# HSoumi/hybrid-als-twotower-recommender

Hardware: AMD Instinct MI355X
Metric: ALS epochs/sec + scored user-item pairs/sec at rank=64, 1/2/4/8 MI355X (higher is better)
Workload: dtype f64

## Files before the change

### hybrid-als-twotower-recommender_amd/csrc/als.hip

```cpp
#include "als_row.h"

namespace hrec {

template <int NT, int CH, int MODE, bool S64 = false, bool IMP = false>
__device__ __forceinline__ void als_row(int64_t row, int lane, const int64_t* __restrict__ indptr,
                                        const int32_t* __restrict__ indices, const float* __restrict__ values,
                                        const float* __restrict__ src, int64_t n_src, int k, double reg,
                                        float* __restrict__ dst, double* __restrict__ lds, double alpha = 0.0,
                                        const double* __restrict__ yty = nullptr) {
  constexpr int KP = 16 * NT;
  const int64_t beg = indptr[row];
  const int64_t end = indptr[row + 1];
  float* __restrict__ out = dst + row * KP;
  if (end == beg) {
    if (lane < KP) out[lane] = 0.f;
    return;
  }
  d4 acc[NT * (NT + 1) / 2];
  double* scratch = lds + RowLds<KP>::kUpPad;
  double* bsh = scratch + 128 + 2 * KP;
  if constexpr (IMP) {
    int n_pos = 0;
    gram_row<NT, CH, MODE, NoHook, S64, true>(beg, end, lane, indices, values, src, n_src, k, reg, acc, bsh, lds,
                                              NoHook(), alpha, yty, &n_pos);
    if (n_pos == 0) {
      if (lane < KP) out[lane] = 0.f;
      return;
    }
  } else {
    gram_row<NT, CH, MODE, NoHook, S64>(beg, end, lane, indices, values, src, n_src, k, reg, acc, bsh, lds);
  }
  factor_row<NT>(lane, acc, lds, scratch, bsh, out);
}

template <int NT, int CH, int MODE, bool S64 = false>
__global__ __launch_bounds__(64, HREC_ALS_WAVES) void als_half_sweep_f64_kernel(
    const int64_t* __restrict__ indptr, const int32_t* __restrict__ indices,
    const float* __restrict__ values, int64_t n_rows, const float* __restrict__ src, int64_t n_src,
    int k, double reg, float* __restrict__ dst) {
  __shared__ __attribute__((aligned(16))) double lds[RowLds<16 * NT>::kSize];
  als_row<NT, CH, MODE, S64>(blockIdx.x, threadIdx.x, indptr, indices, values, src, n_src, k, reg, dst, lds);
}

template <int NT, int CH>
__global__ __launch_bounds__(64, HREC_ALS_WAVES) void als_half_sweep_implicit_kernel(
    const int64_t* __restrict__ indptr, const int32_t* __restrict__ indices,
    const float* __restrict__ values, int64_t n_rows, const float* __restrict__ src, int64_t n_src,
    int k, double reg, double alpha, const double* __restrict__ yty, float* __restrict__ dst) {
  __shared__ __attribute__((aligned(16))) double lds[RowLds<16 * NT>::kSize];
  als_row<NT, CH, 0, false, true>(blockIdx.x, threadIdx.x, indptr, indices, values, src, n_src, k, reg, dst, lds,
                                  alpha, yty);
}

__global__ __launch_bounds__(256) void f32_to_f64_kernel(const float* __restrict__ in, int64_t n,
                                                         double* __restrict__ out) {
  for (int64_t i = (int64_t)blockIdx.x * 256 + threadIdx.x; i < n; i += (int64_t)gridDim.x * 256)
    out[i] = (double)in[i];
}

__global__ __launch_bounds__(256) void transpose_kernel(const float* __restrict__ in, int64_t rows,
                                                        int64_t cols, float* __restrict__ out, int64_t ld_out) {
  __shared__ float tile[64][65];
  const int64_t r0 = (int64_t)blockIdx.x * 64;
  const int64_t c0 = (int64_t)blockIdx.y * 64;
  const int tx = threadIdx.x & 63, ty = threadIdx.x >> 6;
  for (int i = ty; i < 64; i += 4) {
    const int64_t r = r0 + i, c = c0 + tx;
    tile[i][tx] = (r < rows && c < cols) ? in[r * cols + c] : 0.f;
  }
  __syncthreads();
  for (int i = ty; i < 64; i += 4) {
    const int64_t c = c0 + i, r = r0 + tx;
    if (r < rows && c < cols) out[c * ld_out + r] = tile[tx][i];
  }
}

}

using namespace hrec;

extern "C" int hrec_als_half_sweep(const int64_t* indptr, const int32_t* indices, const float* values,
                                   int64_t n_rows, const float* src_factors, int64_t n_src, int k,
                                   int kp, double reg_param, int accum_mode, float* dst_factors,
                                   void* stream) {
  HREC_REQUIRE(hrec_factor_ld_ok(kp), "als_half_sweep: kp must be 16, 32, 64, 96, 128, 192 or 256 (got %d)", kp);
  HREC_REQUIRE(k >= 1 && k <= kp, "als_half_sweep: need 1 <= k <= kp (k=%d kp=%d)", k, kp);
  HREC_REQUIRE(n_rows >= 0 && n_src >= 0, "als_half_sweep: negative size");
  HREC_REQUIRE(n_rows < 0x7fffffffll, "als_half_sweep: too many rows for one launch");
  HREC_REQUIRE(accum_mode == 0 || accum_mode == 1, "als_half_sweep: accum_mode %d unsupported", accum_mode);
  HREC_REQUIRE(reg_param >= 0.0, "als_half_sweep: reg_param must be >= 0");
  if (n_rows == 0) return HREC_OK;
  HREC_REQUIRE(indptr && dst_factors, "als_half_sweep: null pointer");
  HREC_REQUIRE(n_src > 0 && src_factors && indices && values,
               "als_half_sweep: null source factors / CSR arrays");
  HREC_REQUIRE(n_src < 0x7fffffffll, "als_half_sweep: too many source rows for one launch");
  HREC_REQUIRE(kp != 64 || n_src * (int64_t)kp * 4 <= (int64_t)0xffffffffll,
               "als_half_sweep: %lld source rows of %d floats exceed the 4 GiB a gather resource spans; shard the "
               "source side", (long long)n_src, kp);
  if (kp > 64) {
    HREC_REQUIRE(accum_mode == 0, "als_half_sweep: kp > 64 supports accum_mode 0 (f64) only");
    return hrec_als_half_sweep_wide(indptr, indices, values, n_rows, src_factors, n_src, k, kp, reg_param,
                                    dst_factors, stream);
  }
  hipStream_t s = as_stream(stream);
  const dim3 grid((unsigned)n_rows), block(64);
#define HREC_SWEEP(NT, CH, M)                                                                      \
  hipLaunchKernelGGL((als_half_sweep_f64_kernel<NT, CH, M>), grid, block, 0, s, indptr, indices, values, \
                     n_rows, src_factors, n_src, k, reg_param, dst_factors)
  if (accum_mode == 0) {
    if (kp == 64) HREC_SWEEP(4, HREC_ALS_CH0, 0);
    else if (kp == 32) HREC_SWEEP(2, 8, 0);
    else HREC_SWEEP(1, 8, 0);
  } else {
    if (kp == 64) HREC_SWEEP(4, HREC_ALS_CH1, 1);
    else if (kp == 32) HREC_SWEEP(2, 4, 1);
    else HREC_SWEEP(1, 4, 1);
  }
#undef HREC_SWEEP
  return check_launch("als_half_sweep_f64_kernel");
}

extern "C" int hrec_als_half_sweep_implicit(const int64_t* indptr, const int32_t* indices, const float* values,
                                            int64_t n_rows, const float* src_factors, int64_t n_src, int k, int kp,
                                            double reg_param, double alpha, const double* yty, float* dst_factors,
                                            void* stream) {
  HREC_REQUIRE(kp == 16 || kp == 32 || kp == 64,
               "als_half_sweep_implicit: kp must be 16, 32 or 64 (implicit feedback supports rank <= 64; got kp %d)",
// ... 12 lines not shown
               "als_half_sweep_implicit: null source factors / CSR arrays");
  hipStream_t s = as_stream(stream);
  const dim3 grid((unsigned)n_rows), block(64);
#define HREC_SWEEP(NT, CH)                                                                                  \
  hipLaunchKernelGGL((als_half_sweep_implicit_kernel<NT, CH>), grid, block, 0, s, indptr, indices, values, \
                     n_rows, src_factors, n_src, k, reg_param, alpha, yty, dst_factors)
  if (kp == 64) HREC_SWEEP(4, HREC_ALS_CH0);
  else if (kp == 32) HREC_SWEEP(2, 8);
  else HREC_SWEEP(1, 8);
#undef HREC_SWEEP
  return check_launch("als_half_sweep_implicit_kernel");
}

extern "C" int hrec_f32_to_f64(const float* in, int64_t n, double* out, void* stream) {
  HREC_REQUIRE(n >= 0, "f32_to_f64: negative size");
  if (n == 0) return HREC_OK;
  HREC_REQUIRE(in && out, "f32_to_f64: null pointer");
  int64_t blocks = (n + 255) / 256;
  if (blocks > 4096) blocks = 4096;
  hipLaunchKernelGGL(f32_to_f64_kernel, dim3((unsigned)blocks), dim3(256), 0, as_stream(stream), in, n, out);
  return check_launch("f32_to_f64_kernel");
}

extern "C" int hrec_als_half_sweep_src64(const int64_t* indptr, const int32_t* indices, const float* values,
                                         int64_t n_rows, const double* src64, int64_t n_src, int k, int kp,
                                         double reg_param, float* dst_factors, void* stream) {
  HREC_REQUIRE(kp == 64, "als_half_sweep_src64: kp must be 64 (got %d)", kp);
  HREC_REQUIRE(k >= 1 && k <= kp, "als_half_sweep_src64: need 1 <= k <= kp (k=%d kp=%d)", k, kp);
  HREC_REQUIRE(n_rows >= 0 && n_src >= 0, "als_half_sweep_src64: negative size");
  HREC_REQUIRE(n_rows < 0x7fffffffll && n_src < 0x7fffffffll, "als_half_sweep_src64: too many rows for one launch");
  HREC_REQUIRE(n_src * (int64_t)kp * 8 <= (int64_t)0xffffffffll,
               "als_half_sweep_src64: %lld f64 source rows exceed the 4 GiB a gather resource spans", (long long)n_src);
  HREC_REQUIRE(reg_param >= 0.0, "als_half_sweep_src64: reg_param must be >= 0");
  if (n_rows == 0) return HREC_OK;
  HREC_REQUIRE(indptr && dst_factors, "als_half_sweep_src64: null pointer");
  HREC_REQUIRE(n_src > 0 && src64 && indices && values, "als_half_sweep_src64: null source factors / CSR arrays");
  HREC_REQUIRE(((uintptr_t)src64 & 15) == 0, "als_half_sweep_src64: src64 must be 16-B aligned");
  hipLaunchKernelGGL((als_half_sweep_f64_kernel<4, HREC_ALS_CH0, 0, true>), dim3((unsigned)n_rows), dim3(64), 0,
                     as_stream(stream), indptr, indices, values, n_rows, reinterpret_cast<const float*>(src64), n_src,
                     k, reg_param, dst_factors);
  return check_launch("als_half_sweep_f64_kernel (f64 sources)");
}

extern "C" int hrec_transpose_f32(const float* in, int64_t rows, int64_t cols, float* out, int64_t ld_out,
                                  void* stream) {
  HREC_REQUIRE(rows >= 0 && cols >= 0, "transpose: negative size");
  HREC_REQUIRE(ld_out >= rows, "transpose: ld_out < rows");
  if (rows == 0 || cols == 0) return HREC_OK;
  HREC_REQUIRE(in && out, "transpose: null pointer");
  const dim3 grid((unsigned)((rows + 63) / 64), (unsigned)((cols + 63) / 64)), block(256);
  hipLaunchKernelGGL(transpose_kernel, grid, block, 0, as_stream(stream), in, rows, cols, out, ld_out);
  return check_launch("transpose_kernel");
}

#ifdef HREC_ALS_STAMPS
extern "C" int hrec_debug_als_stamps(unsigned long long* host_out, int reset) {
  if (hipMemcpyFromSymbol(host_out, HIP_SYMBOL(g_als_stamps), sizeof(g_als_stamps)) != hipSuccess) return -2;
  if (reset) {
    unsigned long long z[8] = {0};
    if (hipMemcpyToSymbol(HIP_SYMBOL(g_als_stamps), z, sizeof(z)) != hipSuccess) return -2;
  }
  return 0;
}
#endif
// ... 1 lines not shown
```

### hybrid-als-twotower-recommender_amd/csrc/als_row.h

```cpp
#pragma once
#include <type_traits>

#include "common.h"

#ifndef HREC_ALS_WAVES
#define HREC_ALS_WAVES 2
#endif
#ifndef HREC_ALS_CH0
#define HREC_ALS_CH0 8
#endif
#ifndef HREC_ALS_ABLATE
#define HREC_ALS_ABLATE 0
#endif
#ifndef HREC_ALS_SOLVE_UNROLL
#define HREC_ALS_SOLVE_UNROLL 8
#endif
#ifndef HREC_ALS_CH1
#define HREC_ALS_CH1 4
#endif
#ifndef HREC_ALS_INTCVT
#define HREC_ALS_INTCVT 0
#endif
#ifndef HREC_ALS_RLPANEL
#define HREC_ALS_RLPANEL 0
// ... 1 lines not shown
#ifndef HREC_ALS_DIAG4
#define HREC_ALS_DIAG4 3
#endif
#ifndef HREC_ALS_PIPE
#define HREC_ALS_PIPE 1
#endif
#ifndef HREC_ALS_PF
#define HREC_ALS_PF 8
#endif
#ifndef HREC_ALS_PF64
#define HREC_ALS_PF64 4
#endif
#ifndef HREC_ALS_PAIR8
#define HREC_ALS_PAIR8 2
#endif
#ifndef HREC_ALS_ROT1DPP
#define HREC_ALS_ROT1DPP 1
#endif
#ifndef HREC_ALS_ROT1DPP64
#define HREC_ALS_ROT1DPP64 0
#endif
#ifndef HREC_ALS_PR
#define HREC_ALS_PR 2
#endif

namespace hrec {

typedef double d4 __attribute__((ext_vector_type(4)));
typedef hrec_f4 f4;

template <int NT>
struct Vec;
template <>
struct Vec<4> {
  float x[4];
  __device__ static Vec load(const float* p) {
    const float4 t = *reinterpret_cast<const float4*>(p);
    return Vec{{t.x, t.y, t.z, t.w}};
  }
};
template <>
struct Vec<2> {
  float x[2];
  __device__ static Vec load(const float* p) {
    const float2 t = *reinterpret_cast<const float2*>(p);
    return Vec{{t.x, t.y}};
// ... 102 lines not shown
  const long long x = __double_as_longlong(v);
  const int lo = __builtin_amdgcn_readlane((int)x, src);
  const int hi = __builtin_amdgcn_readlane((int)(x >> 32), src);
  return __longlong_as_double(((long long)hi << 32) | (long long)(unsigned)lo);
}

__device__ __forceinline__ void wave_lds_sync() {
  __builtin_amdgcn_fence(__ATOMIC_RELEASE, "wavefront");
  __builtin_amdgcn_wave_barrier();
  __builtin_amdgcn_fence(__ATOMIC_ACQUIRE, "wavefront");
}

template <int KP>
struct RowLds {
  static constexpr int kUp = KP * (KP + 1) / 2;
  static constexpr int kUpPad = ((kUp > 256 ? kUp : 256) + 1) & ~1;
  static constexpr int kSize = kUpPad + 128 + 3 * KP;
};

struct NoHook {
  __device__ void operator()() const {}
};

template <int NT, int CH, int MODE, typename Hook = NoHook, bool S64 = false, bool IMP = false>
__device__ __forceinline__ void gram_row(int64_t beg, int64_t end, int lane, const int32_t* __restrict__ indices,
                                         const float* __restrict__ values, const float* __restrict__ src,
                                         int64_t n_src, int k, double reg, d4 (&acc)[NT * (NT + 1) / 2],
                                         double* __restrict__ bsh, double* __restrict__ stage,
                                         Hook before_lds = Hook(), double alpha = 0.0,
                                         const double* __restrict__ yty = nullptr, int* npos = nullptr) {
  static_assert(!IMP || (MODE == 0 && !S64), "implicit feedback: f64 accumulation of f32 sources only");
  constexpr int KP = 16 * NT;
  constexpr int NPAIR = NT * (NT + 1) / 2;
  constexpr int CHN = 4 * CH;
  const int sub = lane >> 4;
  const int col = lane & 15;
  const int64_t n = end - beg;
  int n_pos = 0;

  STAMP_DECL;
  STAMP(0);
#pragma unroll
  for (int p = 0; p < NPAIR; ++p) acc[p] = d4{0.0, 0.0, 0.0, 0.0};
  if constexpr (HREC_ALS_ABLATE == 4) {
#pragma unroll
    for (int I = 0, p = 0; I < NT; p += NT - I, ++I)
#pragma unroll
      for (int rr = 0; rr < 4; ++rr) acc[p][rr] = (sub + 4 * rr == col) ? 1.0 + reg * (double)n : 0.0;
    if (lane < KP) bsh[lane] = 1.0;
    wave_lds_sync();
    return;
  }
  f4 fa[NPAIR];
  double bp[NT];
#pragma unroll
  for (int t = 0; t < NT; ++t) bp[t] = 0.0;

  auto load_iv = [&](int64_t base, int& ii, float& vv) {
    const int64_t p = base + (lane % CHN);
    const bool ok = (lane < CHN) && (p < end);
    ii = ok ? indices[p] : -1;
    vv = ok ? values[p] : 0.f;
  };
  auto gather = [&](Vec<NT> (&buf)[CH], int ii) {
#pragma unroll
    for (int s = 0; s < CH; ++s) {
      const int idx = __shfl(ii, 4 * s + sub, kWave);
      const int safe = idx < 0 ? 0 : idx;
      Vec<NT> v = Vec<NT>::load(src + (int64_t)safe * KP + NT * col);
#pragma unroll
      for (int t = 0; t < NT; ++t) v.x[t] = idx < 0 ? 0.f : v.x[t];
      buf[s] = v;
    }
  };

  if constexpr (HREC_ALS_PIPE && NT == 4 && !IMP) {
  constexpr int PF = S64 ? HREC_ALS_PF64 : HREC_ALS_PF;
  static_assert(16 % PF == 0, "prefetch distance must divide the window");
  static_assert(!S64 || (NT == 4 && MODE == 0 && (HREC_ALS_DIAG4 == 0 || HREC_ALS_DIAG4 == 3)),
                "f64 sources: kp 64, f64 accumulation only");
  const int voff = (S64 ? 8 : 4) * NT * col;
  const int bp_addr = 4 * sub;
  const uint64_t sbase = (uint64_t)src;
  i4v rsrc;
  rsrc.x = __builtin_amdgcn_readfirstlane((int)(uint32_t)sbase);
  rsrc.y = __builtin_amdgcn_readfirstlane((int)(uint32_t)(sbase >> 32) | ((KP * (S64 ? 8 : 4)) << 16));
  rsrc.z = __builtin_amdgcn_readfirstlane((int)n_src);
  rsrc.w = 0x00020000;
  auto load_win = [&](int64_t w, int& ii, float& vv) {
    const int64_t p = beg + 64 * w + lane;
    const int64_t pc = p < end ? p : end - 1;
    const int iraw = indices[pc];
    const float vraw = values[pc];
    ii = p < end ? iraw : -1;
    vv = p < end ? vraw : 0.f;
  };
  auto bperm = [&](int win, int s) -> int { return __builtin_amdgcn_ds_bpermute(bp_addr + 16 * s, win); };
  const int64_t nsteps = (n + 3) >> 2;
  int iw0, iw1;
  float rw0, rw1;
  load_win(0, iw0, rw0);
  load_win(1, iw1, rw1);
  using RingT = std::conditional_t<S64, VecD, Vec<NT>>;
  auto ring_load = [&](int vi) -> RingT {
    if constexpr (S64) return struct_load_d(rsrc, vi, voff);
    else return struct_load<NT>(rsrc, vi, voff);
  };
  RingT ring[PF];
#pragma unroll
  for (int s = 0; s < PF; ++s) ring[s] = ring_load(bperm(iw0, s));
  int nidx = bperm(iw0, PF);
  constexpr bool kDiag4 = HREC_ALS_DIAG4 && MODE == 0;
  constexpr bool kAhead = HREC_ALS_DIAG4 == 2 && MODE == 0;
  constexpr bool kMemRot = HREC_ALS_DIAG4 == 3 && MODE == 0;
  constexpr int PR = kMemRot ? HREC_ALS_PR : 1;
  constexpr bool kRot1Dpp = kMemRot && (S64 ? HREC_ALS_ROT1DPP64 : HREC_ALS_ROT1DPP);
  static_assert(PR < PF, "rotated loads are issued from the current windows");
  const int voff1 = (S64 ? 8 : 4) * NT * ((col + 4) & 15), voff2 = (S64 ? 8 : 4) * NT * ((col + 8) & 15);
  auto rot_load = [&](int vi, int vo) -> RingT {
    if constexpr (S64) return struct_load_d(rsrc, vi, vo);
    else return struct_load<NT>(rsrc, vi, vo);
  };
  constexpr bool kPairL = kMemRot && HREC_ALS_PAIR8 == 2 && NT == 4;
  using PairT = std::conditional_t<S64, VecD2, Vec<2>>;
  const int hoff = (lane & 8) ? (S64 ? 16 : 8) : 0;
  auto pair_load = [&](int vi, int vo) -> PairT {
    if constexpr (S64) return struct_load_d2(rsrc, vi, vo);
    else return struct_load<2>(rsrc, vi, vo);
  };
  RingT rot1[PR], rot2[PR];
  PairT rotA[PR], rotB[PR];
  if constexpr (kMemRot) {
#pragma unroll
    for (int q = 0; q < PR; ++q) {
      const int vi = bperm(iw0, q);
      if constexpr (!kRot1Dpp) rot1[q] = rot_load(vi, voff1);
      if constexpr (kPairL) {
        rotA[q] = pair_load(vi, voff + hoff);
        rotB[q] = pair_load(vi, voff2 + hoff);
// ... 134 lines not shown
            }
          } else {
            fa[p] = __builtin_amdgcn_mfma_f32_16x16x4f32(cur.x[I], cur.x[J], fa[p], 0, 0, 0);
          }
          ++p;
        }
      }
#pragma unroll
      for (int t = 0; t < NT; ++t) bp[t] = fma(rv, a[t], bp[t]);
      if (MODE == 1 && ((s % HREC_ALS_CH1) == HREC_ALS_CH1 - 1 || s + 1 == rem)) {
#pragma unroll
        for (int p2 = 0; p2 < NPAIR; ++p2) {
#pragma unroll
          for (int rr = 0; rr < 4; ++rr) acc[p2][rr] += (double)fa[p2][rr];
        }
      }
    }
    if (stop || 16 * (w + 1) >= nsteps) break;
    iw0 = iw1;
    rw0 = rw1;
    iw1 = iw2;
    rw1 = rw2;
  }
  if constexpr (kDiag4) {
    const int i4 = lane >> 4, q4 = (lane >> 2) & 3, j4 = lane & 3;
#pragma unroll
    for (int I = 0, p = 0; I < NT; p += NT - I, ++I) {
#pragma unroll
      for (int sh = 0; sh < 3; ++sh) {
        const int r = 4 * q4 + i4, c = 4 * ((q4 + sh) & 3) + j4;
        if (kPair8 && sh == 2) {
          const bool mine = kPairL ? (q4 >= 2) == (I >= 2) : (q4 >= 2) == (I % 2 == 1);
          const double v = kPairL ? dc[I & 1] : dc[I / 2];
          stage[mine ? r * 16 + c : 256] = v;
          stage[mine ? c * 16 + r : 257] = v;
          continue;
        }
        stage[r * 16 + c] = dg[I][sh];
        stage[c * 16 + r] = dg[I][sh];
      }
      wave_lds_sync();
#pragma unroll
      for (int rr = 0; rr < 4; ++rr) acc[p][rr] = stage[(sub + 4 * rr) * 16 + col];
      wave_lds_sync();
    }
  }
// ... 97 lines not shown
#pragma unroll
      for (int J = I; J < NT; ++J) {
#pragma unroll
        for (int rr = 0; rr < 4; ++rr) acc[p][rr] += yty[(NT * (sub + 4 * rr) + I) * KP + NT * col + J];
        ++p;
      }
    }
    *npos = n_pos;
  }
  const double lambda = (double)(IMP ? (int64_t)n_pos : n) * reg;
  {
    int p = 0;
#pragma unroll
    for (int I = 0; I < NT; ++I) {
#pragma unroll
      for (int rr = 0; rr < 4; ++rr) {
        if (sub + 4 * rr == col) acc[p][rr] += (NT * col + I < k) ? lambda : 1.0;
      }
      p += NT - I;
    }
  }
}

template <int NT>
__device__ __forceinline__ void factor_row(int lane, d4 (&acc)[NT * (NT + 1) / 2], double* __restrict__ Up,
                                           double* __restrict__ scratch, const double* __restrict__ bsh,
                                           float* __restrict__ out) {
  constexpr int KP = 16 * NT;
  constexpr int NPAIR = NT * (NT + 1) / 2;
  double* __restrict__ colbuf = scratch;
  double* __restrict__ dsh = colbuf + 128;
  double* __restrict__ rdsh = dsh + KP;
  const int sub = lane >> 4, col = lane & 15;
  STAMP_DECL;
  STAMP(0);
  if constexpr (HREC_ALS_ABLATE == 1) {
    double sum = 0.0;
#pragma unroll
    for (int p = 0; p < NPAIR; ++p) sum += acc[p][0] + acc[p][1] + acc[p][2] + acc[p][3];
    wave_lds_sync();
    if (lane < KP) out[lane] = (float)(sum + bsh[lane]);
    return;
  }
  auto pidx = [](int I, int K) { return I * NT - (I * (I - 1)) / 2 + (K - I); };
  double bs = 0.0;
#pragma unroll
  for (int J = 0; J < NT; ++J) {
#pragma unroll
    for (int K = J; K < NT; ++K) {
#pragma unroll
      for (int rr = 0; rr < 4; ++rr) {
        const int q = 16 * J + sub + 4 * rr, c = 16 * K + col;
        if (q <= c) Up[tri(c) + q] = acc[pidx(J, K)][rr];
      }
    }
    wave_lds_sync();
    if (J == 0) bs = lane < KP ? bsh[lane] : 0.0;
    const int c = lane;
    const bool own = c >= 16 * J && c < KP;
    double a[16];
#pragma unroll
    for (int m = 0; m < 16; ++m) {
      const int q = 16 * J + m;
      if constexpr (HREC_ALS_RLPANEL) {
        a[m] = !own ? 0.0 : q <= c ? Up[tri(c) + q] : c < 16 * J + 16 ? Up[tri(q) + c] : 0.0;
      } else {
        a[m] = (own && q <= c) ? Up[tri(c) + q] : 0.0;
      }
    }
    double piv = bcast(a[0], 16 * J);
    if constexpr (HREC_ALS_RLPANEL) {
#pragma unroll
      for (int i = 0; i < 16; ++i) {
        const int pv = 16 * J + i;
        double u[16];
#pragma unroll
        for (int m0 = i + 1; m0 < 16; ++m0) u[m0] = bcast(a[m0], pv);
        const double r0 = __builtin_amdgcn_rcp(piv);
        const double r = fma(r0, fma(-piv, r0, 1.0), r0);
// ... 46 lines not shown
          if (!kRl2 || m0 > i) a[m0 + 1] = fma(-u.y, ut, a[m0 + 1]);
        }
      }
    }
    wave_lds_sync();
    if (J + 1 < NT) {
      double dq[4];
#pragma unroll
      for (int rr = 0; rr < 4; ++rr) dq[rr] = dsh[16 * J + sub + 4 * rr];
      d4 yv[NT];
#pragma unroll
      for (int K = J + 1; K < NT; ++K) {
#pragma unroll
        for (int rr = 0; rr < 4; ++rr) {
          const double x = Up[tri(16 * K + col) + 16 * J + sub + 4 * rr];
          acc[pidx(J, K)][rr] = x;
          yv[K][rr] = x * dq[rr];
        }
      }
#pragma unroll
      for (int K = J + 1; K < NT; ++K) {
#pragma unroll
        for (int M = K; M < NT; ++M) {
#pragma unroll
          for (int rr = 0; rr < 4; ++rr)
            acc[pidx(K, M)] = __builtin_amdgcn_mfma_f64_16x16x4f64(-acc[pidx(J, K)][rr], yv[M][rr],
                                                                    acc[pidx(K, M)], 0, 0, 0);
        }
      }
    }
  }
  STAMP(3);
  const int lc = lane < KP ? lane : KP - 1;
  const double myrd = rdsh[lc];
  if constexpr (HREC_ALS_ABLATE == 3) {
    if (lane < KP) out[lane] = (float)(myrd + Up[tri(lane)]);
    return;
  }
  double bi = bs * myrd;
#pragma unroll HREC_ALS_SOLVE_UNROLL
  for (int q = KP - 1; q >= 0; --q) {
    const double u = Up[tri(q) + (lane < KP ? lane : 0)];
    const double xq = bcast(bi, q);
    if (lane < q) bi = fma(-u, xq, bi);
  }
  STAMP(4);
  if (lane < KP) out[NT * (lane & 15) + (lane >> 4)] = (float)bi;
  wave_lds_sync();
}

}
```

### hybrid-als-twotower-recommender_amd/src/_hrec.py

```python
import ctypes
import os

import torch

_HERE = os.path.dirname(os.path.abspath(__file__))
LIB_PATH = os.environ.get("HREC_LIB") or os.path.join(os.path.dirname(_HERE), "lib", "libhrec.so")

_c_i32 = ctypes.c_int
_c_i64 = ctypes.c_int64
_c_u64 = ctypes.c_uint64
_c_dbl = ctypes.c_double
_c_sz = ctypes.c_size_t
_vp = ctypes.c_void_p

_SIGNATURES = {
    "hrec_abi_version": (_c_i32, []),
    "hrec_last_error": (ctypes.c_char_p, []),
    "hrec_synth_row_counts": (_c_i32, [_c_u64, _c_u64, _c_i64, _c_i64, _c_i64, _c_i32, _vp, _vp]),
    "hrec_synth_fill": (_c_i32, [_c_u64, _c_u64, _c_u64, _c_i64, _c_i64, _c_i64, _c_i32, _c_i32,
                                 _vp, _vp, _vp, _vp]),
    "hrec_scan_workspace_bytes": (_c_sz, [_c_i64]),
    "hrec_exclusive_scan_i64": (_c_i32, [_vp, _c_i64, _vp, _vp, _c_sz, _vp]),
    "hrec_encode_ids_workspace_bytes": (_c_sz, [_c_i64]),
    "hrec_encode_ids": (_c_i32, [_vp, _c_i64, _c_i64, _c_i64, _vp, _vp, _vp, _vp, _c_sz, _vp]),
    "hrec_encode_ids_ex": (_c_i32, [_vp, _c_i64, _c_i64, _c_i64, _vp, _vp, _vp, _vp, _vp, _vp, _c_sz, _vp]),
    "hrec_minmax_i64_workspace_bytes": (_c_sz, [_c_i64]),
    "hrec_minmax_i64": (_c_i32, [_vp, _c_i64, _vp, _vp, _c_sz, _vp]),
    "hrec_coo_to_csr_workspace_bytes": (_c_sz, [_c_i64, _c_i64]),
    "hrec_coo_to_csr": (_c_i32, [_vp, _vp, _vp, _c_i64, _c_i64, _vp, _vp, _vp, _vp, _c_sz, _vp]),
    "hrec_remap_i32": (_c_i32, [_vp, _c_i64, _vp, _c_i64, _vp]),
    "hrec_rows_descending_pairs": (_c_i32, [_vp, _c_i64, _vp, _vp]),
    "hrec_coo_to_csr_sorted": (_c_i32, [_vp, _vp, _vp, _c_i64, _c_i64, _vp, _vp, _vp, _vp]),
    "hrec_als_init_factors": (_c_i32, [_c_u64, _c_i64, _c_i64, _c_i32, _c_i32, _vp, _vp]),
    "hrec_als_half_sweep_src64": (_c_i32, [_vp, _vp, _vp, _c_i64, _vp, _c_i64, _c_i32, _c_i32, _c_dbl, _vp, _vp]),
    "hrec_f32_to_f64": (_c_i32, [_vp, _c_i64, _vp, _vp]),
    "hrec_als_gramian_workspace_bytes": (_c_sz, [_c_i64, _c_i32]),
    "hrec_als_gramian": (_c_i32, [_vp, _c_i64, _c_i32, _c_i32, _vp, _vp, _c_sz, _vp]),
    "hrec_als_half_sweep_implicit": (_c_i32, [_vp, _vp, _vp, _c_i64, _vp, _c_i64, _c_i32, _c_i32, _c_dbl, _c_dbl,
                                              _vp, _vp, _vp]),
    "hrec_als_half_sweep_nonneg": (_c_i32, [_vp, _vp, _vp, _c_i64, _vp, _c_i64, _c_i32, _c_i32, _c_dbl, _c_i32,
                                            _c_dbl, _vp, _vp, _vp, _vp]),
    "hrec_als_half_sweep": (_c_i32, [_vp, _vp, _vp, _c_i64, _vp, _c_i64, _c_i32, _c_i32, _c_dbl,
                                     _c_i32, _vp, _vp]),
    "hrec_transpose_f32": (_c_i32, [_vp, _c_i64, _c_i64, _vp, _c_i64, _vp]),
    "hrec_als_score": (_c_i32, [_vp, _vp, _c_i32, _vp, _c_i64, _vp, _c_i64, _c_i32, _c_i32, _vp,
                                _vp]),
    "hrec_als_score_topk_workspace_bytes": (_c_sz, [_c_i32, _c_i64, _c_i32]),
    "hrec_als_score_topk": (_c_i32, [_vp, _vp, _c_i32, _vp, _c_i64, _c_i64, _c_i32, _c_i32, _c_i32, _vp, _vp, _vp,
                                     _vp, _c_sz, _vp]),
    "hrec_als_items_bf16_bytes": (_c_sz, [_c_i64, _c_i32]),
    "hrec_als_items_bf16": (_c_i32, [_vp, _c_i64, _c_i64, _c_i32, _vp, _c_sz, _vp]),
    "hrec_als_score_topk_pruned_workspace_bytes": (_c_sz, [_c_i32, _c_i64, _c_i32, _c_i32]),
    "hrec_als_score_topk_pruned": (_c_i32, [_vp, _vp, _c_i32, _vp, _c_i64, _vp, _c_i64, _vp, _c_i64, _c_i32,
                                            _c_i32, _c_i32, _vp, _vp, _vp, _vp, _c_sz, _vp]),
    "hrec_als_score_topk_pruned_counts": (_c_i32, [_vp, _c_i32, _c_i64, _c_i32, _c_i32, _vp, _vp]),
    "hrec_topk_workspace_bytes": (_c_sz, [_c_i64, _c_i64, _c_i32, _c_i32]),
    "hrec_topk_f32": (_c_i32, [_vp, _c_i64, _c_i64, _c_i64, _c_i32, _vp, _vp, _vp, _c_sz, _vp]),
# ... 241 lines not shown
            nnz, n_rows, _dev(indptr, torch.int64, "indptr"), _dev(indices, torch.int32, "indices"),
            _dev(values, torch.float32, "values"), _stream()))
        return indptr, indices, values
    ws = torch.empty(max(int(lib().hrec_coo_to_csr_workspace_bytes(nnz, n_rows)), 16), dtype=torch.uint8,
                     device=dev)
    _check("hrec_coo_to_csr", lib().hrec_coo_to_csr(
        _dev(rows, torch.int32, "rows"), _dev(cols, torch.int32, "cols"), _dev(vals, torch.float32, "vals"),
        nnz, n_rows, _dev(indptr, torch.int64, "indptr"), _dev(indices, torch.int32, "indices"),
        _dev(values, torch.float32, "values"), _dev(ws, torch.uint8, "ws"), ws.numel(), _stream()))
    return indptr, indices, values


def remap_i32(x, table):
    _check("hrec_remap_i32", lib().hrec_remap_i32(
        _dev(x, torch.int32, "x"), x.numel(), _dev(table, torch.int32, "table"), table.numel(), _stream()))
    return x


def als_init_factors(seed, row_begin, n_rows, k, kp, out):
    _check("hrec_als_init_factors", lib().hrec_als_init_factors(
        seed, row_begin, n_rows, k, kp, _dev(out, torch.float32, "out"), _stream()))


def als_half_sweep(indptr, indices, values, src_factors, k, reg_param, dst_factors, accum_mode=0, src64=None):
    n_rows = indptr.numel() - 1
    kp = dst_factors.shape[1]
    if src_factors.shape[1] != kp or dst_factors.shape[0] < n_rows:
        raise HrecError("als_half_sweep: factor shapes do not match")
    if src64 is not None:
        if accum_mode != 0 or src64.shape != src_factors.shape:
            raise HrecError("als_half_sweep: src64 needs accum_mode 0 and the source factors' shape")
        _check("hrec_als_half_sweep_src64", lib().hrec_als_half_sweep_src64(
            _dev(indptr, torch.int64, "indptr"), _dev(indices, torch.int32, "indices"),
            _dev(values, torch.float32, "values"), n_rows, _dev(src64, torch.float64, "src64"),
            src64.shape[0], k, kp, float(reg_param), _dev(dst_factors, torch.float32, "dst_factors"), _stream()))
        return
    _check("hrec_als_half_sweep", lib().hrec_als_half_sweep(
        _dev(indptr, torch.int64, "indptr"), _dev(indices, torch.int32, "indices"),
        _dev(values, torch.float32, "values"), n_rows,
        _dev(src_factors, torch.float32, "src_factors"), src_factors.shape[0], k, kp,
        float(reg_param), int(accum_mode), _dev(dst_factors, torch.float32, "dst_factors"),
        _stream()))


def als_gramian(src_factors, k):
    n_src, kp = src_factors.shape
    dev = src_factors.device
    out = torch.empty((kp, kp), dtype=torch.float64, device=dev)
    need = int(lib().hrec_als_gramian_workspace_bytes(n_src, kp))
    ws = torch.empty(max(need, 16), dtype=torch.uint8, device=dev)
    _check("hrec_als_gramian", lib().hrec_als_gramian(
# ... 785 lines not shown
```

### hybrid-als-twotower-recommender_amd/src/als_engine.py

```python
import math
import os

import torch
import torch.distributed as dist

from . import _hrec
from .synthetic import DeviceCSR


SRC64_MAX_BYTES = int(os.environ.get("HREC_ALS_SRC64_MB", "128")) << 20


def padded_k(k):
    if k <= 16:
        return 16
    if k <= 32:
        return 32
    for kp in (64, 96, 128, 192, 256):
        if k <= kp:
            return kp
    raise ValueError(f"rank {k} > 256 is not supported by the half-sweep kernels")


def shard_range(n, world, rank):
    per = math.ceil(n / world) if n else 0
    return rank * per, per


def shard_chunks(n, world, rank, chunks):
    per = math.ceil(n / world) if n else 0
    cs = math.ceil(per / chunks) if per else 0
    return [(c * world * cs + rank * cs, cs) for c in range(chunks)], cs

# ... 161 lines not shown

    def _gather(self, full, local):
        if self.world > 1:
            dist.all_gather_into_tensor(full, local, group=self.group)

    def _src64(self, src):
        if not self._src64_ok or src.numel() * 8 > SRC64_MAX_BYTES:
            return None
        if self._s64 is None or self._s64.numel() < src.numel():
            self._s64 = torch.empty(src.numel(), dtype=torch.float64, device=src.device)
        out = self._s64[: src.numel()].view(src.shape)
        return _hrec.f32_to_f64(src, out)

    def _launcher(self, src):
        if self.nonnegative:
            yty = self.gramian(src, self.k) if self.implicit else None
            return lambda ip, ix, v, dst: self.sweep(ip, ix, v, src, self.k, self.reg, dst, implicit=self.implicit,
                                                     alpha=self.alpha if self.implicit else 0.0, yty=yty)
        if self.implicit:
            yty = self.gramian(src, self.k)
            return lambda ip, ix, v, dst: self.sweep(ip, ix, v, src, self.k, self.reg, self.alpha, yty, dst)
        s64 = self._src64(src)
        extra = {} if s64 is None else {"src64": s64}
        return lambda ip, ix, v, dst: self.sweep(ip, ix, v, src, self.k, self.reg, dst, self.accum_mode, **extra)

    def _sweep(self, csr, src, local, full, cs, chunks):
        launch = self._launcher(src)
        if chunks == 1:
            launch(csr.indptr, csr.indices, csr.values, local)
            self._gather(full, local)
            return
        W = self.world
        compute = torch.cuda.current_stream() if self.comm is not None else None
        for c in range(chunks):
            rows = slice(c * cs, (c + 1) * cs)
            launch(csr.indptr[c * cs: (c + 1) * cs + 1], csr.indices, csr.values, local[rows])
            out = full[c * W * cs: (c + 1) * W * cs]
            if self.comm is None:
                dist.all_gather_into_tensor(out, local[rows], group=self.group)
                continue
            done = torch.cuda.Event()
            done.record(compute)
            with torch.cuda.stream(self.comm):
                self.comm.wait_event(done)
                dist.all_gather_into_tensor(out, local[rows], group=self.group)
        if self.comm is not None:
# ... 43 lines not shown
```

### include/hrec.h

```cpp
#ifndef HREC_H
#define HREC_H

#include <stddef.h>
#include <stdint.h>

#ifdef __cplusplus
extern "C" {
#endif

#define HREC_ABI_VERSION 7

#define HREC_OK 0
#define HREC_E_INVALID (-1)
#define HREC_E_LAUNCH (-2)
#define HREC_E_UNSUPPORTED (-3)

int hrec_abi_version(void);
const char* hrec_last_error(void);

int hrec_synth_row_counts(uint64_t seed, uint64_t threshold, int64_t row_begin,
                          int64_t n_rows, int64_t n_cols, int transposed,
                          int64_t* counts, void* stream);
int hrec_synth_fill(uint64_t seed, uint64_t seed2, uint64_t threshold,
                    int64_t row_begin, int64_t n_rows, int64_t n_cols,
// ... 22 lines not shown
int hrec_coo_to_csr(const int32_t* rows, const int32_t* cols, const float* vals,
                    int64_t nnz, int64_t n_rows, int64_t* indptr, int32_t* indices,
                    float* values, void* workspace, size_t workspace_bytes,
                    void* stream);
int hrec_rows_descending_pairs(const int32_t* rows, int64_t n, int32_t* out, void* stream);
int hrec_coo_to_csr_sorted(const int32_t* rows, const int32_t* cols, const float* vals,
                           int64_t nnz, int64_t n_rows, int64_t* indptr, int32_t* indices,
                           float* values, void* stream);

int hrec_remap_i32(int32_t* x, int64_t n, const int32_t* table, int64_t table_n, void* stream);

int hrec_als_init_factors(uint64_t seed, int64_t row_begin, int64_t n_rows,
                          int k, int kp, float* out, void* stream);

int hrec_als_half_sweep(const int64_t* indptr, const int32_t* indices,
                        const float* values, int64_t n_rows,
                        const float* src_factors, int64_t n_src, int k, int kp,
                        double reg_param, int accum_mode, float* dst_factors,
                        void* stream);

int hrec_als_half_sweep_src64(const int64_t* indptr, const int32_t* indices, const float* values,
                              int64_t n_rows, const double* src64, int64_t n_src, int k, int kp,
                              double reg_param, float* dst_factors, void* stream);
int hrec_f32_to_f64(const float* in, int64_t n, double* out, void* stream);

size_t hrec_als_gramian_workspace_bytes(int64_t n_src, int kp);
int hrec_als_gramian(const float* src_factors, int64_t n_src, int k, int kp,
                     double* yty, void* workspace, size_t workspace_bytes,
                     void* stream);

int hrec_als_half_sweep_implicit(const int64_t* indptr, const int32_t* indices, const float* values,
                                 int64_t n_rows, const float* src_factors, int64_t n_src, int k, int kp,
                                 double reg_param, double alpha, const double* yty, float* dst_factors,
                                 void* stream);

int hrec_als_half_sweep_nonneg(const int64_t* indptr, const int32_t* indices, const float* values,
                               int64_t n_rows, const float* src_factors, int64_t n_src, int k, int kp,
                               double reg_param, int implicit, double alpha, const double* yty,
                               float* dst_factors, int32_t* iters_out, void* stream);

int hrec_transpose_f32(const float* in, int64_t rows, int64_t cols, float* out,
                       int64_t ld_out, void* stream);

int hrec_als_score(const float* user_factors, const int64_t* user_rows,
                   int n_users, const float* item_factors_t, int64_t ld_items,
                   const int64_t* item_rows, int64_t n_items, int k, int kp,
// ... 225 lines not shown
```

Baseline: 12.98.

## Add persistent pooled ALS half-sweep kernel with shared LDS slice pool

Adds a persistent kernel for the kp=64 f64-accumulation half sweep. Each workgroup of 12 waves pulls rows from a global atomic ticket and shares 8 LDS slices among its waves. A slice is taken only after the Gram accumulation finishes, and the factorization writes trailing updates to LDS instead of holding them in registers. The aim is to raise wave occupancy beyond what a full per-wave LDS allocation allows and to balance uneven row lengths. The cost is spin-waiting on slices, atomic traffic, and extra LDS round trips during the factorization. The pooled path is the default for sweeps of at least 65536 rows, and an explicit kernel selector API is added.

Result: faster. 13.16 (median of 6 runs) (+1.3%).

```diff
diff --git a/hybrid-als-twotower-recommender_amd/csrc/als.hip b/hybrid-als-twotower-recommender_amd/csrc/als.hip
--- a/hybrid-als-twotower-recommender_amd/csrc/als.hip
+++ b/hybrid-als-twotower-recommender_amd/csrc/als.hip
@@ -1,3 +1,5 @@
+#include <mutex>
+
 #include "als_row.h"
 
 namespace hrec {
@@ -42,6 +44,104 @@
   als_row<NT, CH, MODE, S64>(blockIdx.x, threadIdx.x, indptr, indices, values, src, n_src, k, reg, dst, lds);
 }
 
+#ifndef HREC_ALS_POOL_LATE
+#define HREC_ALS_POOL_LATE 1
+#endif
+#ifndef HREC_ALS_POOL_PRIO
+#define HREC_ALS_POOL_PRIO 0
+#endif
+#ifndef HREC_ALS_POOL_LDSG
+#define HREC_ALS_POOL_LDSG 1
+#endif
+#ifndef HREC_ALS_POOL_ANY32
+#define HREC_ALS_POOL_ANY32 0
+#endif
+#ifndef HREC_ALS_POOL_ANY64
+#define HREC_ALS_POOL_ANY64 1
+#endif
+#ifndef HREC_ALS_POOL_SLEEP
+#define HREC_ALS_POOL_SLEEP 8
+#endif
+constexpr int kPoolWaves = 12, kPoolSlices = 8;
+constexpr size_t kPoolLdsBytes = (size_t)kPoolSlices * RowLds<64>::kSize * sizeof(double);
+
+template <bool ANY>
+__device__ __forceinline__ int slice_acquire(int* busy, int cls, int lane) {
+  int slot, zero = 0;
+  asm volatile("" : "+v"(zero));
+  for (;;) {
+    int got = -1;
+    if (lane == 0) {
+      for (int i = 0; i < (ANY ? kPoolSlices : 2) && got < 0; ++i) {
+        const int sl = (2 * cls + i) % kPoolSlices;
+        if (atomicCAS(&busy[sl], zero, 1) == 0) got = sl;
+      }
+    }
+    slot = __builtin_amdgcn_readfirstlane(got);
+    if (slot >= 0) break;
+    __builtin_amdgcn_s_sleep(HREC_ALS_POOL_SLEEP);
+  }
+  __builtin_amdgcn_fence(__ATOMIC_ACQUIRE, "workgroup");
+  if constexpr (HREC_ALS_POOL_PRIO) __builtin_amdgcn_s_setprio(HREC_ALS_POOL_PRIO);
+  return slot;
+}
+
+__device__ __forceinline__ void slice_release(int* busy, int slot, int lane) {
+  __builtin_amdgcn_fence(__ATOMIC_RELEASE, "workgroup");
+  if (lane == 0) atomicExch(&busy[slot], 0);
+  if constexpr (HREC_ALS_POOL_PRIO) __builtin_amdgcn_s_setprio(0);
+}
+
+template <bool S64>
+__global__ __launch_bounds__(64 * kPoolWaves, 3) void als_half_sweep_f64_kernel_pooled(
+    const int64_t* __restrict__ indptr, const int32_t* __restrict__ indices, const float* __restrict__ values,
+    int64_t n_rows, const float* __restrict__ src, int64_t n_src, int k, double reg, float* __restrict__ dst,
+    unsigned* __restrict__ ticket) {
+  constexpr int NT = 4, KP = 64;
+  extern __shared__ __attribute__((aligned(16))) double pool[];
+  __shared__ int busy[kPoolSlices];
+  if (threadIdx.x < kPoolSlices) busy[threadIdx.x] = 0;
+  __syncthreads();
+  const int lane = threadIdx.x & 63;
+  const int cls = __builtin_amdgcn_readfirstlane((int)(threadIdx.x >> 6)) & 3;
+  for (;;) {
+    unsigned t = 0;
+    if (lane == 0) t = atomicAdd(ticket, 1u);
+    const int64_t row = (int64_t)(unsigned)__builtin_amdgcn_readfirstlane((int)t);
+    if (row >= n_rows) return;
+    const int64_t beg = indptr[row];
+    const int64_t end = indptr[row + 1];
+    float* __restrict__ out = dst + row * KP;
+    if (end == beg) {
+      if (lane < KP) out[lane] = 0.f;
+      continue;
+    }
+    int gl = lane, fl = lane;
+    asm volatile("" : "+v"(gl));
+    d4 acc[NT * (NT + 1) / 2];
+    int slot = -1;
+    auto acquire = [&]() -> double* {
+      slot = slice_acquire<S64 ? HREC_ALS_POOL_ANY64 != 0 : HREC_ALS_POOL_ANY32 != 0>(busy, cls, lane);
+      return pool + slot * RowLds<KP>::kSize;
+    };
+    double* lds = nullptr;
+    if constexpr (HREC_ALS_POOL_LATE) {
+      gram_row<NT, HREC_ALS_CH0, 0, NoHook, S64, false, true>(beg, end, gl, indices, values, src, n_src, k, reg, acc,
+                                                         nullptr, nullptr, NoHook(), 0.0, nullptr, nullptr, acquire);
+      lds = pool + slot * RowLds<KP>::kSize;
+    } else {
+      lds = acquire();
+      gram_row<NT, HREC_ALS_CH0, 0, NoHook, S64, false, true>(beg, end, gl, indices, values, src, n_src, k, reg, acc,
+                                                 lds + RowLds<KP>::kUpPad + 128 + 2 * KP, lds);
+    }
+    double* scratch = lds + RowLds<KP>::kUpPad;
+    asm volatile("" : "+v"(fl));
+    if constexpr (HREC_ALS_POOL_LDSG) factor_row_lds<NT>(fl, acc, lds, scratch, scratch + 128 + 2 * KP, out);
+    else factor_row<NT>(fl, acc, lds, scratch, scratch + 128 + 2 * KP, out);
+    slice_release(busy, slot, lane);
+  }
+}
+
 template <int NT, int CH>
 __global__ __launch_bounds__(64, HREC_ALS_WAVES) void als_half_sweep_implicit_kernel(
     const int64_t* __restrict__ indptr, const int32_t* __restrict__ indices,
@@ -78,6 +178,66 @@
 }
 
 using namespace hrec;
+
+namespace {
+
+constexpr int kTicketRing = 4096;
+constexpr int kMaxDevices = 64;
+
+struct PoolDevice {
+  unsigned* ring = nullptr;
+  unsigned next = 0;
+  int cus = 0;
+};
+
+int pooled_ticket(unsigned** word, int* cus) {
+  static std::mutex mu;
+  static PoolDevice devs[kMaxDevices];
+  int dev = 0;
+  if (hipGetDevice(&dev) != hipSuccess || dev < 0 || dev >= kMaxDevices) {
+    set_error("als_half_sweep (pooled): no current device");
+    return HREC_E_LAUNCH;
+  }
+  std::lock_guard<std::mutex> lock(mu);
+  PoolDevice& d = devs[dev];
+  if (!d.ring) {
+    if (hipDeviceGetAttribute(&d.cus, hipDeviceAttributeMultiprocessorCount, dev) != hipSuccess || d.cus < 1 ||
+        hipMalloc(&d.ring, kTicketRing * sizeof(unsigned)) != hipSuccess) {
+      d.ring = nullptr;
+      return check_launch("als_half_sweep (pooled): ticket words");
+    }
+  }
+  *word = d.ring + (d.next++ % kTicketRing);
+  *cus = d.cus;
+  return HREC_OK;
+}
+
+template <bool S64>
+int launch_pooled(const int64_t* indptr, const int32_t* indices, const float* values, int64_t n_rows,
+                  const float* src, int64_t n_src, int k, double reg, float* dst, hipStream_t s) {
+  auto kfn = als_half_sweep_f64_kernel_pooled<S64>;
+  if (!allow_max_lds(kfn)) return check_launch("als_half_sweep_f64_kernel_pooled: LDS attribute");
+  unsigned* ticket = nullptr;
+  int cus = 0;
+  const int rc = pooled_ticket(&ticket, &cus);
+  if (rc != HREC_OK) return rc;
+  if (hipMemsetAsync(ticket, 0, sizeof(unsigned), s) != hipSuccess)
+    return check_launch("als_half_sweep_f64_kernel_pooled: memset");
+  const int64_t need = (n_rows + kPoolWaves - 1) / kPoolWaves;
+  const dim3 grid((unsigned)(need < cus ? need : cus)), block(64 * kPoolWaves);
+  hipLaunchKernelGGL(kfn, grid, block, kPoolLdsBytes, s, indptr, indices, values, n_rows, src, n_src, k, reg, dst,
+                     ticket);
+  return check_launch("als_half_sweep_f64_kernel_pooled");
+}
+
+constexpr int64_t kPooledMinRows = 65536;
+constexpr bool kPooledF32 = true;
+constexpr bool kPooledF64 = true;
+inline int pick_kernel(bool s64, int64_t n_rows) {
+  return (s64 ? kPooledF64 : kPooledF32) && n_rows >= kPooledMinRows ? 1 : 0;
+}
+
+}
 
 extern "C" int hrec_als_half_sweep(const int64_t* indptr, const int32_t* indices, const float* values,
                                    int64_t n_rows, const float* src_factors, int64_t n_src, int k,
@@ -103,6 +263,8 @@
                                     dst_factors, stream);
   }
   hipStream_t s = as_stream(stream);
+  if (kp == 64 && accum_mode == 0 && pick_kernel(false, n_rows) == 1)
+    return launch_pooled<false>(indptr, indices, values, n_rows, src_factors, n_src, k, reg_param, dst_factors, s);
   const dim3 grid((unsigned)n_rows), block(64);
 #define HREC_SWEEP(NT, CH, M)                                                                      \
   hipLaunchKernelGGL((als_half_sweep_f64_kernel<NT, CH, M>), grid, block, 0, s, indptr, indices, values, \
@@ -161,24 +323,62 @@
   return check_launch("f32_to_f64_kernel");
 }
 
-extern "C" int hrec_als_half_sweep_src64(const int64_t* indptr, const int32_t* indices, const float* values,
-                                         int64_t n_rows, const double* src64, int64_t n_src, int k, int kp,
-                                         double reg_param, float* dst_factors, void* stream) {
-  HREC_REQUIRE(kp == 64, "als_half_sweep_src64: kp must be 64 (got %d)", kp);
-  HREC_REQUIRE(k >= 1 && k <= kp, "als_half_sweep_src64: need 1 <= k <= kp (k=%d kp=%d)", k, kp);
-  HREC_REQUIRE(n_rows >= 0 && n_src >= 0, "als_half_sweep_src64: negative size");
-  HREC_REQUIRE(n_rows < 0x7fffffffll && n_src < 0x7fffffffll, "als_half_sweep_src64: too many rows for one launch");
+static int half_sweep_src64(const char* name, const int64_t* indptr, const int32_t* indices, const float* values,
+                            int64_t n_rows, const double* src64, int64_t n_src, int k, int kp, double reg_param,
+                            int kernel, float* dst_factors, void* stream) {
+  HREC_REQUIRE(kp == 64, "%s: kp must be 64 (got %d)", name, kp);
+  HREC_REQUIRE(k >= 1 && k <= kp, "%s: need 1 <= k <= kp (k=%d kp=%d)", name, k, kp);
+  HREC_REQUIRE(n_rows >= 0 && n_src >= 0, "%s: negative size", name);
+  HREC_REQUIRE(n_rows < 0x7fffffffll && n_src < 0x7fffffffll, "%s: too many rows for one launch", name);
   HREC_REQUIRE(n_src * (int64_t)kp * 8 <= (int64_t)0xffffffffll,
-               "als_half_sweep_src64: %lld f64 source rows exceed the 4 GiB a gather resource spans", (long long)n_src);
-  HREC_REQUIRE(reg_param >= 0.0, "als_half_sweep_src64: reg_param must be >= 0");
+               "%s: %lld f64 source rows exceed the 4 GiB a gather resource spans", name, (long long)n_src);
+  HREC_REQUIRE(reg_param >= 0.0, "%s: reg_param must be >= 0", name);
   if (n_rows == 0) return HREC_OK;
-  HREC_REQUIRE(indptr && dst_factors, "als_half_sweep_src64: null pointer");
-  HREC_REQUIRE(n_src > 0 && src64 && indices && values, "als_half_sweep_src64: null source factors / CSR arrays");
-  HREC_REQUIRE(((uintptr_t)src64 & 15) == 0, "als_half_sweep_src64: src64 must be 16-B aligned");
+  HREC_REQUIRE(indptr && dst_factors, "%s: null pointer", name);
+  HREC_REQUIRE(n_src > 0 && src64 && indices && values, "%s: null source factors / CSR arrays", name);
+  HREC_REQUIRE(((uintptr_t)src64 & 15) == 0, "%s: src64 must be 16-B aligned", name);
+  if (kernel < 0) kernel = pick_kernel(true, n_rows);
+  if (kernel == 1)
+    return launch_pooled<true>(indptr, indices, values, n_rows, reinterpret_cast<const float*>(src64), n_src, k,
+                               reg_param, dst_factors, as_stream(stream));
   hipLaunchKernelGGL((als_half_sweep_f64_kernel<4, HREC_ALS_CH0, 0, true>), dim3((unsigned)n_rows), dim3(64), 0,
                      as_stream(stream), indptr, indices, values, n_rows, reinterpret_cast<const float*>(src64), n_src,
                      k, reg_param, dst_factors);
   return check_launch("als_half_sweep_f64_kernel (f64 sources)");
+}
+
+extern "C" int hrec_als_half_sweep_src64(const int64_t* indptr, const int32_t* indices, const float* values,
+                                         int64_t n_rows, const double* src64, int64_t n_src, int k, int kp,
+                                         double reg_param, float* dst_factors, void* stream) {
+  return half_sweep_src64("als_half_sweep_src64", indptr, indices, values, n_rows, src64, n_src, k, kp, reg_param, -1,
+                          dst_factors, stream);
+}
+
+extern "C" int hrec_als_half_sweep_kernel(const int64_t* indptr, const int32_t* indices, const float* values,
+                                          int64_t n_rows, const void* src, int src_f64, int64_t n_src, int k, int kp,
+                                          double reg_param, int kernel, float* dst_factors, void* stream) {
+  HREC_REQUIRE(kernel == 0 || kernel == 1, "als_half_sweep_kernel: kernel must be 0 (one wave per row) or 1 (pooled), got %d",
+               kernel);
+  HREC_REQUIRE(kp == 64, "als_half_sweep_kernel: kp must be 64 (got %d)", kp);
+  if (src_f64)
+    return half_sweep_src64("als_half_sweep_kernel", indptr, indices, values, n_rows, static_cast<const double*>(src),
+                            n_src, k, kp, reg_param, kernel, dst_factors, stream);
+  HREC_REQUIRE(k >= 1 && k <= kp, "als_half_sweep_kernel: need 1 <= k <= kp (k=%d kp=%d)", k, kp);
+  HREC_REQUIRE(n_rows >= 0 && n_src >= 0, "als_half_sweep_kernel: negative size");
+  HREC_REQUIRE(n_rows < 0x7fffffffll && n_src < 0x7fffffffll, "als_half_sweep_kernel: too many rows for one launch");
+  HREC_REQUIRE(n_src * (int64_t)kp * 4 <= (int64_t)0xffffffffll,
+               "als_half_sweep_kernel: %lld source rows exceed the 4 GiB a gather resource spans", (long long)n_src);
+  HREC_REQUIRE(reg_param >= 0.0, "als_half_sweep_kernel: reg_param must be >= 0");
+  if (n_rows == 0) return HREC_OK;
+  HREC_REQUIRE(indptr && dst_factors, "als_half_sweep_kernel: null pointer");
+  HREC_REQUIRE(n_src > 0 && src && indices && values, "als_half_sweep_kernel: null source factors / CSR arrays");
+  const float* src32 = static_cast<const float*>(src);
+  if (kernel == 1)
+    return launch_pooled<false>(indptr, indices, values, n_rows, src32, n_src, k, reg_param, dst_factors,
+                                as_stream(stream));
+  hipLaunchKernelGGL((als_half_sweep_f64_kernel<4, HREC_ALS_CH0, 0>), dim3((unsigned)n_rows), dim3(64), 0,
+                     as_stream(stream), indptr, indices, values, n_rows, src32, n_src, k, reg_param, dst_factors);
+  return check_launch("als_half_sweep_f64_kernel");
 }
 
 extern "C" int hrec_transpose_f32(const float* in, int64_t rows, int64_t cols, float* out, int64_t ld_out,
diff --git a/hybrid-als-twotower-recommender_amd/csrc/als_row.h b/hybrid-als-twotower-recommender_amd/csrc/als_row.h
--- a/hybrid-als-twotower-recommender_amd/csrc/als_row.h
+++ b/hybrid-als-twotower-recommender_amd/csrc/als_row.h
@@ -47,6 +47,15 @@
 #endif
 #ifndef HREC_ALS_PR
 #define HREC_ALS_PR 2
+#endif
+#ifndef HREC_ALS_POOL_PF
+#define HREC_ALS_POOL_PF 8
+#endif
+#ifndef HREC_ALS_POOL_PF64
+#define HREC_ALS_POOL_PF64 4
+#endif
+#ifndef HREC_ALS_POOL_ROT1DPP64
+#define HREC_ALS_POOL_ROT1DPP64 1
 #endif
 
 namespace hrec {
@@ -195,13 +204,18 @@
   __device__ void operator()() const {}
 };
 
-template <int NT, int CH, int MODE, typename Hook = NoHook, bool S64 = false, bool IMP = false>
+template <int NT, int CH, int MODE, typename Hook = NoHook, bool S64 = false, bool IMP = false,
+          bool POOLED = false, typename Acq = NoHook>
 __device__ __forceinline__ void gram_row(int64_t beg, int64_t end, int lane, const int32_t* __restrict__ indices,
                                          const float* __restrict__ values, const float* __restrict__ src,
                                          int64_t n_src, int k, double reg, d4 (&acc)[NT * (NT + 1) / 2],
                                          double* __restrict__ bsh, double* __restrict__ stage,
                                          Hook before_lds = Hook(), double alpha = 0.0,
-                                         const double* __restrict__ yty = nullptr, int* npos = nullptr) {
+                                         const double* __restrict__ yty = nullptr, int* npos = nullptr,
+                                         Acq acquire = Acq()) {
+  constexpr bool kAcq = !std::is_same_v<Acq, NoHook>;
+  static_assert(!kAcq || (HREC_ALS_PIPE && NT == 4 && !IMP && HREC_ALS_ABLATE != 4),
+                "late slice acquisition: the kp-64 ring pipeline only");
   static_assert(!IMP || (MODE == 0 && !S64), "implicit feedback: f64 accumulation of f32 sources only");
   constexpr int KP = 16 * NT;
   constexpr int NPAIR = NT * (NT + 1) / 2;
@@ -248,7 +262,7 @@
   };
 
   if constexpr (HREC_ALS_PIPE && NT == 4 && !IMP) {
-  constexpr int PF = S64 ? HREC_ALS_PF64 : HREC_ALS_PF;
+  constexpr int PF = POOLED ? (S64 ? HREC_ALS_POOL_PF64 : HREC_ALS_POOL_PF) : (S64 ? HREC_ALS_PF64 : HREC_ALS_PF);
   static_assert(16 % PF == 0, "prefetch distance must divide the window");
   static_assert(!S64 || (NT == 4 && MODE == 0 && (HREC_ALS_DIAG4 == 0 || HREC_ALS_DIAG4 == 3)),
                 "f64 sources: kp 64, f64 accumulation only");
@@ -287,7 +301,8 @@
   constexpr bool kAhead = HREC_ALS_DIAG4 == 2 && MODE == 0;
   constexpr bool kMemRot = HREC_ALS_DIAG4 == 3 && MODE == 0;
   constexpr int PR = kMemRot ? HREC_ALS_PR : 1;
-  constexpr bool kRot1Dpp = kMemRot && (S64 ? HREC_ALS_ROT1DPP64 : HREC_ALS_ROT1DPP);
+  constexpr bool kRot1Dpp =
+      kMemRot && (S64 ? (POOLED ? HREC_ALS_POOL_ROT1DPP64 : HREC_ALS_ROT1DPP64) : HREC_ALS_ROT1DPP);
   static_assert(PR < PF, "rotated loads are issued from the current windows");
   const int voff1 = (S64 ? 8 : 4) * NT * ((col + 4) & 15), voff2 = (S64 ? 8 : 4) * NT * ((col + 8) & 15);
   auto rot_load = [&](int vi, int vo) -> RingT {
@@ -468,6 +483,11 @@
     iw1 = iw2;
     rw1 = rw2;
   }
+  if constexpr (kAcq) {
+    double* base = acquire();
+    stage = base;
+    bsh = base + RowLds<KP>::kUpPad + 128 + 2 * KP;
+  }
   if constexpr (kDiag4) {
     const int i4 = lane >> 4, q4 = (lane >> 2) & 3, j4 = lane & 3;
 #pragma unroll
@@ -611,8 +631,8 @@
   }
 }
 
-template <int NT>
-__device__ __forceinline__ void factor_row(int lane, d4 (&acc)[NT * (NT + 1) / 2], double* __restrict__ Up,
+template <int NT, bool LDSG>
+__device__ __forceinline__ void factor_row_impl(int lane, d4 (&acc)[NT * (NT + 1) / 2], double* __restrict__ Up,
                                            double* __restrict__ scratch, const double* __restrict__ bsh,
                                            float* __restrict__ out) {
   constexpr int KP = 16 * NT;
@@ -635,15 +655,20 @@
   double bs = 0.0;
 #pragma unroll
   for (int J = 0; J < NT; ++J) {
-#pragma unroll
-    for (int K = J; K < NT; ++K) {
-#pragma unroll
-      for (int rr = 0; rr < 4; ++rr) {
-        const int q = 16 * J + sub + 4 * rr, c = 16 * K + col;
-        if (q <= c) Up[tri(c) + q] = acc[pidx(J, K)][rr];
-      }
-    }
-    wave_lds_sync();
+    if (!LDSG || J == 0) {
+#pragma unroll
+      for (int I = J; I < (LDSG ? NT : J + 1); ++I) {
+#pragma unroll
+        for (int K = I; K < NT; ++K) {
+#pragma unroll
+          for (int rr = 0; rr < 4; ++rr) {
+            const int q = 16 * I + sub + 4 * rr, c = 16 * K + col;
+            if (q <= c) Up[tri(c) + q] = acc[pidx(I, K)][rr];
+          }
+        }
+      }
+      wave_lds_sync();
+    }
     if (J == 0) bs = lane < KP ? bsh[lane] : 0.0;
     const int c = lane;
     const bool own = c >= 16 * J && c < KP;
@@ -736,12 +761,27 @@
       for (int K = J + 1; K < NT; ++K) {
 #pragma unroll
         for (int M = K; M < NT; ++M) {
-#pragma unroll
-          for (int rr = 0; rr < 4; ++rr)
-            acc[pidx(K, M)] = __builtin_amdgcn_mfma_f64_16x16x4f64(-acc[pidx(J, K)][rr], yv[M][rr],
-                                                                    acc[pidx(K, M)], 0, 0, 0);
-        }
-      }
+          if constexpr (LDSG) {
+            d4 t;
+#pragma unroll
+            for (int rr = 0; rr < 4; ++rr) t[rr] = Up[tri(16 * M + col) + 16 * K + sub + 4 * rr];
+#pragma unroll
+            for (int rr = 0; rr < 4; ++rr)
+              t = __builtin_amdgcn_mfma_f64_16x16x4f64(-acc[pidx(J, K)][rr], yv[M][rr], t, 0, 0, 0);
+#pragma unroll
+            for (int rr = 0; rr < 4; ++rr) {
+              const int q = 16 * K + sub + 4 * rr, c = 16 * M + col;
+              if (q <= c) Up[tri(c) + q] = t[rr];
+            }
+          } else {
+#pragma unroll
+            for (int rr = 0; rr < 4; ++rr)
+              acc[pidx(K, M)] = __builtin_amdgcn_mfma_f64_16x16x4f64(-acc[pidx(J, K)][rr], yv[M][rr],
+                                                                      acc[pidx(K, M)], 0, 0, 0);
+          }
+        }
+      }
+      if constexpr (LDSG) wave_lds_sync();
     }
   }
   STAMP(3);
@@ -763,4 +803,18 @@
   wave_lds_sync();
 }
 
-}
+template <int NT>
+__device__ __forceinline__ void factor_row(int lane, d4 (&acc)[NT * (NT + 1) / 2], double* __restrict__ Up,
+                                           double* __restrict__ scratch, const double* __restrict__ bsh,
+                                           float* __restrict__ out) {
+  factor_row_impl<NT, false>(lane, acc, Up, scratch, bsh, out);
+}
+
+template <int NT>
+__device__ __forceinline__ void factor_row_lds(int lane, d4 (&acc)[NT * (NT + 1) / 2], double* __restrict__ Up,
+                                               double* __restrict__ scratch, const double* __restrict__ bsh,
+                                               float* __restrict__ out) {
+  factor_row_impl<NT, true>(lane, acc, Up, scratch, bsh, out);
+}
+
+}
diff --git a/hybrid-als-twotower-recommender_amd/src/_hrec.py b/hybrid-als-twotower-recommender_amd/src/_hrec.py
--- a/hybrid-als-twotower-recommender_amd/src/_hrec.py
+++ b/hybrid-als-twotower-recommender_amd/src/_hrec.py
@@ -33,6 +33,8 @@
     "hrec_coo_to_csr_sorted": (_c_i32, [_vp, _vp, _vp, _c_i64, _c_i64, _vp, _vp, _vp, _vp]),
     "hrec_als_init_factors": (_c_i32, [_c_u64, _c_i64, _c_i64, _c_i32, _c_i32, _vp, _vp]),
     "hrec_als_half_sweep_src64": (_c_i32, [_vp, _vp, _vp, _c_i64, _vp, _c_i64, _c_i32, _c_i32, _c_dbl, _vp, _vp]),
+    "hrec_als_half_sweep_kernel": (_c_i32, [_vp, _vp, _vp, _c_i64, _vp, _c_i32, _c_i64, _c_i32, _c_i32, _c_dbl, _c_i32,
+                                            _vp, _vp]),
     "hrec_f32_to_f64": (_c_i32, [_vp, _c_i64, _vp, _vp]),
     "hrec_als_gramian_workspace_bytes": (_c_sz, [_c_i64, _c_i32]),
     "hrec_als_gramian": (_c_i32, [_vp, _c_i64, _c_i32, _c_i32, _vp, _vp, _c_sz, _vp]),
@@ -320,11 +322,23 @@
         seed, row_begin, n_rows, k, kp, _dev(out, torch.float32, "out"), _stream()))
 
 
-def als_half_sweep(indptr, indices, values, src_factors, k, reg_param, dst_factors, accum_mode=0, src64=None):
+def als_half_sweep(indptr, indices, values, src_factors, k, reg_param, dst_factors, accum_mode=0, src64=None,
+                   kernel=None):
     n_rows = indptr.numel() - 1
     kp = dst_factors.shape[1]
     if src_factors.shape[1] != kp or dst_factors.shape[0] < n_rows:
         raise HrecError("als_half_sweep: factor shapes do not match")
+    if kernel is not None:
+        if accum_mode != 0 or kp != 64:
+            raise HrecError("als_half_sweep: an explicit kernel needs kp 64 and accum_mode 0")
+        if src64 is not None and src64.shape != src_factors.shape:
+            raise HrecError("als_half_sweep: src64 needs the source factors' shape")
+        src = _dev(src_factors, torch.float32, "src_factors") if src64 is None else _dev(src64, torch.float64, "src64")
+        _check("hrec_als_half_sweep_kernel", lib().hrec_als_half_sweep_kernel(
+            _dev(indptr, torch.int64, "indptr"), _dev(indices, torch.int32, "indices"),
+            _dev(values, torch.float32, "values"), n_rows, src, 0 if src64 is None else 1, src_factors.shape[0], k,
+            kp, float(reg_param), int(kernel), _dev(dst_factors, torch.float32, "dst_factors"), _stream()))
+        return
     if src64 is not None:
         if accum_mode != 0 or src64.shape != src_factors.shape:
             raise HrecError("als_half_sweep: src64 needs accum_mode 0 and the source factors' shape")
diff --git a/hybrid-als-twotower-recommender_amd/src/als_engine.py b/hybrid-als-twotower-recommender_amd/src/als_engine.py
--- a/hybrid-als-twotower-recommender_amd/src/als_engine.py
+++ b/hybrid-als-twotower-recommender_amd/src/als_engine.py
@@ -9,6 +9,7 @@
 
 
 SRC64_MAX_BYTES = int(os.environ.get("HREC_ALS_SRC64_MB", "128")) << 20
+HALF_SWEEP_KERNEL = {"": None, "0": 0, "1": 1}[os.environ.get("HREC_ALS_KERNEL", "")]
 
 
 def padded_k(k):
@@ -216,6 +217,8 @@
             return lambda ip, ix, v, dst: self.sweep(ip, ix, v, src, self.k, self.reg, self.alpha, yty, dst)
         s64 = self._src64(src)
         extra = {} if s64 is None else {"src64": s64}
+        if HALF_SWEEP_KERNEL is not None and self._src64_ok:
+            extra["kernel"] = HALF_SWEEP_KERNEL
         return lambda ip, ix, v, dst: self.sweep(ip, ix, v, src, self.k, self.reg, dst, self.accum_mode, **extra)
 
     def _sweep(self, csr, src, local, full, cs, chunks):
diff --git a/include/hrec.h b/include/hrec.h
--- a/include/hrec.h
+++ b/include/hrec.h
@@ -68,6 +68,9 @@
 int hrec_als_half_sweep_src64(const int64_t* indptr, const int32_t* indices, const float* values,
                               int64_t n_rows, const double* src64, int64_t n_src, int k, int kp,
                               double reg_param, float* dst_factors, void* stream);
+int hrec_als_half_sweep_kernel(const int64_t* indptr, const int32_t* indices, const float* values,
+                               int64_t n_rows, const void* src, int src_f64, int64_t n_src, int k, int kp,
+                               double reg_param, int kernel, float* dst_factors, void* stream);
 int hrec_f32_to_f64(const float* in, int64_t n, double* out, void* stream);
 
 size_t hrec_als_gramian_workspace_bytes(int64_t n_src, int kp);
```
